# jianwang-mpi/GlobalEgoMocap

Hardware: AMD Instinct MI355X
Metric: optimised windows/sec (10-frame, 15-joint) (higher is better)
Workload: dtype f32

## Files before the change

globalegomocap_amd/csrc/gemm_f32.hip:

```cpp
#include <cstdio>
#include <cstdlib>

#include "gem_internal.h"
#include "gemm_glds.h"
#include "gemm_rows.h"

namespace gem {

typedef float f32x16 __attribute__((ext_vector_type(16)));
typedef float f32x4 __attribute__((ext_vector_type(4)));
typedef int i32x8 __attribute__((ext_vector_type(8)));

constexpr int BK_MIN = 32;

#ifdef GEM_TRACE
__device__ long long* g_gemm_trace = nullptr;
#define GEM_TRACE_MARK(slot_)                                                                            \
    if (g_gemm_trace && threadIdx.x == 0)                                                                \
        g_gemm_trace[4 * (blockIdx.x + gridDim.x * (blockIdx.y + gridDim.y * blockIdx.z)) + (slot_)] = wall_clock64();
#else
#define GEM_TRACE_MARK(slot_)
#endif

template <int TAPS, int EPI, int RM, int RN, int TAG, int BK>
__global__ __launch_bounds__(256) void gemm_f32_kernel(const float* __restrict__ A, int lda,
                                                       const float* __restrict__ W,
                                                       const float* __restrict__ bias,
                                                       const float* __restrict__ aux, float* __restrict__ C,
                                                       int ldc, int M, int N, int K, int T, int tiles_per_slice,
                                                       size_t slab_stride, const int* __restrict__ m_dev,
                                                       const int* __restrict__ row_map, int dyn_W) {
    constexpr int BM = 64 * RM, BN = 64 * RN;
    constexpr int LDS_LD = BK + 4;
    constexpr int TPR = BK / 4;
    constexpr int RPP = 256 / TPR;
    constexpr int A_LD4 = BM / RPP;
    constexpr int B_LD4 = BN / RPP;
    extern __shared__ __attribute__((aligned(16))) float lds[];
    constexpr int BUF = (BM + BN) * LDS_LD;

    const int tid = threadIdx.x;
    const int lane = tid & 63, wave = tid >> 6;
    const int wm = wave >> 1, wn = wave & 1;
    GEM_TRACE_MARK(0);
    int m0 = blockIdx.y * BM, n0 = blockIdx.x * BN;
    if (m_dev) M = *m_dev;
    const int kTiles = K / BK;
    bool split = gridDim.z > 1;
    int kt_begin = blockIdx.z * tiles_per_slice;
    int kt_end = min(TAPS * kTiles, kt_begin + tiles_per_slice);
    if (dyn_W > 0) {
        if (M <= 0) return;
        const int CT = N / BN;
        const DynSplit d = dyn_split(M, BM, CT, dyn_W, TAPS * kTiles, ldc);
        const int id = blockIdx.x + gridDim.x * (blockIdx.y + gridDim.y * blockIdx.z);
        if (id >= CT * d.RT * d.SK) return;
        const int ks = id / (CT * d.RT);
        n0 = (id % CT) * BN;
        m0 = ((id / CT) % d.RT) * BM;
        kt_begin = ks * d.per;
        kt_end = min(TAPS * kTiles, kt_begin + d.per);
        split = true;
        C += (size_t)ks * d.slab;
    } else {
        if (m0 >= M) return;
        if (split) C += (size_t)blockIdx.z * slab_stride;
    }

    const int c4 = (tid % TPR) * 4;
    const int lrow = tid / TPR;
    static_assert(A_LD4 <= 8, "row tables hold up to 8 entries");
    i32x8 a_row, a_t, a_src;
#pragma unroll
    for (int i = 0; i < A_LD4; ++i) {
        const int r_ = m0 + lrow + RPP * i;
        a_row[i] = r_;
        a_t[i] = (TAPS == 3) ? (r_ % T) : 0;
        int s_ = r_;
        if (TAPS == 1 && row_map) s_ = row_map[r_ < M ? r_ : 0];
        a_src[i] = s_;
    }
    f32x4 ra[A_LD4], rb[B_LD4];
    bool a_ok[A_LD4];

#define GEM_LOAD_TILE(kt_)                                                                                   \
    {                                                                                                        \
        const int tap_ = (TAPS == 3) ? ((kt_) >= kTiles) + ((kt_) >= 2 * kTiles) : 0;                                                      \
        const int k0_ = ((kt_) - tap_ * kTiles) * BK + c4;                                                   \
        _Pragma("unroll") for (int i = 0; i < A_LD4; ++i) {                                                  \
            bool ok_ = a_row[i] < M;                                                                         \
            if (TAPS == 3) {                                                                                 \
                const int tt_ = a_t[i] + tap_ - 1;                                                           \
                ok_ = ok_ && tt_ >= 0 && tt_ < T;                                                            \
            }                                                                                                \
            const int src_ = ok_ ? a_src[i] + ((TAPS == 3) ? tap_ - 1 : 0) : 0;                               \
            ra[i] = *reinterpret_cast<const f32x4*>(A + (size_t)src_ * lda + k0_);                           \
            a_ok[i] = ok_;   \
        }                                                                                                    \
        const float* Wt_ = W + (size_t)tap_ * N * K;                                                         \
        _Pragma("unroll") for (int i = 0; i < B_LD4; ++i)                                                    \
            rb[i] = *reinterpret_cast<const f32x4*>(Wt_ + (size_t)(n0 + lrow + RPP * i) * K + k0_);          \
    }
#define GEM_STORE_TILE(buf_)                                                                                 \
    {                                                                                                        \
        _Pragma("unroll") for (int i = 0; i < A_LD4; ++i)                                                    \
            *reinterpret_cast<f32x4*>(lds + (buf_) * BUF + (lrow + RPP * i) * LDS_LD + c4) =                  \
                a_ok[i] ? ra[i] : f32x4{0.f, 0.f, 0.f, 0.f};                                                 \
        _Pragma("unroll") for (int i = 0; i < B_LD4; ++i)                                                    \
            *reinterpret_cast<f32x4*>(lds + (buf_) * BUF + (BM + lrow + RPP * i) * LDS_LD + c4) = rb[i];      \
    }

    f32x16 acc[RM][RN];
#pragma unroll
    for (int i = 0; i < RM; ++i)
#pragma unroll
        for (int j = 0; j < RN; ++j)
#pragma unroll
            for (int e = 0; e < 16; ++e) acc[i][j][e] = 0.f;

    const int fr = lane & 31, fh = lane >> 5;
    constexpr bool DBUF = (RM * RN > 1);
    GEM_LOAD_TILE(kt_begin);
    GEM_STORE_TILE(0);
    __syncthreads();
    GEM_TRACE_MARK(1);
    int cur = 0;
#ifndef GEM_ABLATE
#define GEM_ABLATE 0
#endif
    for (int kt = kt_begin; kt < kt_end; ++kt) {
        const bool more = kt + 1 < kt_end;
        if (more && GEM_ABLATE < 1) GEM_LOAD_TILE(kt + 1);
        const float* as = lds + cur * BUF + (wm * 32 * RM + fr) * LDS_LD + fh * (BK / 2);
        const float* bs = lds + cur * BUF + (BM + wn * 32 * RN + fr) * LDS_LD + fh * (BK / 2);
        if (RM * RN == 1 && GEM_ABLATE == 0) {
            f32x4 av[BK / 8], bv[BK / 8];
#pragma unroll
            for (int q = 0; q < BK / 8; ++q) {
                av[q] = *reinterpret_cast<const f32x4*>(as + 4 * q);
                bv[q] = *reinterpret_cast<const f32x4*>(bs + 4 * q);
            }
            __builtin_amdgcn_sched_barrier(0);
#pragma unroll
            for (int q = 0; q < BK / 8; ++q) {
                acc[0][0] = __builtin_amdgcn_mfma_f32_32x32x2f32(av[q].x, bv[q].x, acc[0][0], 0, 0, 0);
                acc[0][0] = __builtin_amdgcn_mfma_f32_32x32x2f32(av[q].y, bv[q].y, acc[0][0], 0, 0, 0);
                acc[0][0] = __builtin_amdgcn_mfma_f32_32x32x2f32(av[q].z, bv[q].z, acc[0][0], 0, 0, 0);
                acc[0][0] = __builtin_amdgcn_mfma_f32_32x32x2f32(av[q].w, bv[q].w, acc[0][0], 0, 0, 0);
            }
        } else {
#pragma unroll
        for (int q = 0; q < BK / 8; ++q) {
            f32x4 av[RM], bv[RN];
#pragma unroll
            for (int i = 0; i < RM; ++i) av[i] = *reinterpret_cast<const f32x4*>(as + i * 32 * LDS_LD + 4 * (GEM_ABLATE >= 3 ? 0 : q));
#pragma unroll
            for (int j = 0; j < RN; ++j) bv[j] = *reinterpret_cast<const f32x4*>(bs + j * 32 * LDS_LD + 4 * (GEM_ABLATE >= 3 ? 0 : q));
            if (GEM_ABLATE >= 3) {
#pragma unroll
                for (int i = 0; i < RM; ++i) asm volatile("" : "+v"(av[i]));
            }
#pragma unroll
            for (int i = 0; i < RM; ++i)
#pragma unroll
                for (int j = 0; j < RN; ++j) {
                    acc[i][j] = __builtin_amdgcn_mfma_f32_32x32x2f32(av[i].x, bv[j].x, acc[i][j], 0, 0, 0);
                    acc[i][j] = __builtin_amdgcn_mfma_f32_32x32x2f32(av[i].y, bv[j].y, acc[i][j], 0, 0, 0);
                    acc[i][j] = __builtin_amdgcn_mfma_f32_32x32x2f32(av[i].z, bv[j].z, acc[i][j], 0, 0, 0);
                    acc[i][j] = __builtin_amdgcn_mfma_f32_32x32x2f32(av[i].w, bv[j].w, acc[i][j], 0, 0, 0);
                }
        }
        }
        if (GEM_ABLATE >= 2) continue;
        if (DBUF) {
            if (more) GEM_STORE_TILE(cur ^ 1);
            __syncthreads();
            cur ^= 1;
        } else {
            __syncthreads();
            if (more) GEM_STORE_TILE(0);
            __syncthreads();
        }
    }
#undef GEM_LOAD_TILE
#undef GEM_STORE_TILE
    GEM_TRACE_MARK(2);

#pragma unroll
    for (int i = 0; i < RM; ++i)
#pragma unroll
        for (int j = 0; j < RN; ++j) {
            const int col = n0 + wn * 32 * RN + j * 32 + fr;
            float bv = 0.f;
            if ((EPI == EPI_BIAS || EPI == EPI_BIAS_LRELU) && !split) bv = bias[col];
#pragma unroll
            for (int e = 0; e < 16; ++e) {
                const int row = m0 + wm * 32 * RM + i * 32 + (e & 3) + 8 * (e >> 2) + 4 * fh;
                if (row < M) {
                    float v = acc[i][j][e] + bv;
                    if (EPI == EPI_BIAS_LRELU && !split) v = v > 0.f ? v : v * LEAKY_SLOPE;
                    if (EPI == EPI_MASK && !split) v *= (aux[(size_t)row * ldc + col] > 0.f) ? 1.f : LEAKY_SLOPE;
                    C[(size_t)row * ldc + col] = v;
                }
            }
        }
    GEM_TRACE_MARK(3);
}

template <int EPI>
__global__ __launch_bounds__(256) void splitk_reduce_kernel(const float* __restrict__ slabs, int nslab, size_t slab_stride,
                                                            const float* __restrict__ bias, const float* __restrict__ aux,
                                                            float* __restrict__ C, int M, int N, int ldc,
                                                            const int* __restrict__ m_dev, int dyn_W, int n_tiles) {
    if (m_dev) M = *m_dev;
    if (dyn_W > 0) {
        const DynSplit d = dyn_split(M, 64, N / 64, dyn_W, n_tiles, ldc);
        nslab = d.SK;
        slab_stride = d.slab;
    }
    const int n4 = N / 4;
    const size_t i = (size_t)blockIdx.x * 256 + threadIdx.x;
    if (i >= (size_t)M * n4) return;
    const int row = (int)(i / n4), c = (int)(i - (size_t)row * n4) * 4;
    const size_t off = (size_t)row * ldc + c;
    f32x4 v = *reinterpret_cast<const f32x4*>(slabs + off);
    for (int z = 1; z < nslab; ++z) v += *reinterpret_cast<const f32x4*>(slabs + (size_t)z * slab_stride + off);
    if (EPI == EPI_BIAS || EPI == EPI_BIAS_LRELU) v += *reinterpret_cast<const f32x4*>(bias + c);
    if (EPI == EPI_BIAS_LRELU) {
#pragma unroll
        for (int q = 0; q < 4; ++q) v[q] = v[q] > 0.f ? v[q] : v[q] * LEAKY_SLOPE;
    }
    if (EPI == EPI_MASK) {
        const f32x4 m = *reinterpret_cast<const f32x4*>(aux + off);
#pragma unroll
        for (int q = 0; q < 4; ++q) v[q] *= m[q] > 0.f ? 1.f : LEAKY_SLOPE;
    }
    *reinterpret_cast<f32x4*>(C + off) = v;
}

constexpr int LDS_PER_CU = 160 * 1024;
int pick_splitk(const gem_handle* h, long blocks, int n_tiles, size_t slab_elems) {
    const int N_CU = h->n_cu;
    if (!h->ws.splitk || blocks >= 3 * N_CU) return 1;
    int best = 1;
    double best_score = -1.0;
    for (int sk = 1; sk <= 8; ++sk) {
        if (sk > 1 && (n_tiles / sk < 6 || (size_t)sk * slab_elems > h->ws.splitk_elems)) break;
        const long wgs = blocks * sk;
        const long per_cu = (wgs + N_CU - 1) / N_CU;
        double score = (double)wgs / (double)(per_cu * N_CU);
        if (per_cu < 2) score *= 0.6;
        score -= 0.01 * sk;
        if (score > best_score) { best_score = score; best = sk; }
    }
    return best;
}

int launch_splitk_reduce(gem_handle* h, int epi, int nslab, size_t slab, const float* bias, const float* aux, float* C, int M, int N,
                         int ldc, const int* m_dev, hipStream_t s, int dyn_W, int n_tiles) {
    const size_t n4 = (size_t)M * (N / 4);
    const dim3 grid((unsigned)((n4 + 255) / 256));
    switch (epi) {
        case EPI_BIAS: hipLaunchKernelGGL(splitk_reduce_kernel<EPI_BIAS>, grid, dim3(256), 0, s, h->ws.splitk, nslab, slab, bias, aux, C, M, N, ldc, m_dev, dyn_W, n_tiles); break;
        case EPI_BIAS_LRELU: hipLaunchKernelGGL(splitk_reduce_kernel<EPI_BIAS_LRELU>, grid, dim3(256), 0, s, h->ws.splitk, nslab, slab, bias, aux, C, M, N, ldc, m_dev, dyn_W, n_tiles); break;
        case EPI_MASK: hipLaunchKernelGGL(splitk_reduce_kernel<EPI_MASK>, grid, dim3(256), 0, s, h->ws.splitk, nslab, slab, bias, aux, C, M, N, ldc, m_dev, dyn_W, n_tiles); break;
        default: hipLaunchKernelGGL(splitk_reduce_kernel<EPI_NONE>, grid, dim3(256), 0, s, h->ws.splitk, nslab, slab, bias, aux, C, M, N, ldc, m_dev, dyn_W, n_tiles); break;
    }
    GEM_HIP(hipGetLastError());
    return 0;
}

template <int TAPS, int EPI, int RM, int RN, int TAG, int BK>
static int launch_one(gem_handle* h, const Layer& L, const float* A, int lda, const float* aux, float* C, int ldc, int M, int T,
                      hipStream_t s, const int* row_map) {
    const int* m_dev = h->ws.dyn ? h->ws.n_active + (TAPS == 3 ? 1 : 0) : nullptr;
    constexpr int BM = 64 * RM, BN = 64 * RN;
    size_t shmem = (RM * RN > 1 ? 2 : 1) * (size_t)(BM + BN) * (BK + 4) * sizeof(float);
    auto k = gemm_f32_kernel<TAPS, EPI, RM, RN, TAG, BK>;
    static PerDeviceOnce attr_once;
    if (attr_once.need(h->cfg.device)) {
        GEM_HIP(hipFuncSetAttribute(reinterpret_cast<const void*>(k), hipFuncAttributeMaxDynamicSharedMemorySize, LDS_PER_CU));
    }
    const int n_tiles = TAPS * (L.K / BK);
    dim3 grid(L.N / BN, (M + BM - 1) / BM, 1);
    const size_t slab = (size_t)M * ldc;
    const int sk = pick_splitk(h, (long)grid.x * grid.y, n_tiles, slab);
    const int per = (n_tiles + sk - 1) / sk;
    grid.z = (n_tiles + per - 1) / per;
    const long wgs = (long)grid.x * grid.y * grid.z;
    const long per_cu = (wgs + h->n_cu - 1) / h->n_cu;
    if (per_cu <= 8) {
        const size_t want = (((size_t)LDS_PER_CU - 8192) / per_cu) & ~(size_t)1023;
        if (want > shmem) shmem = want;
    }
    const bool dyn = m_dev && RM * RN == 1 && grid.z > 1 && (size_t)wgs * 64 * BN <= h->ws.splitk_elems;
    if (grid.z == 1) {
        note_kernel(h, reinterpret_cast<const void*>(k));
        hipLaunchKernelGGL(k, grid, dim3(256), shmem, s, A, lda, L.w, L.bias, aux, C, ldc, M, L.N, L.K, T, n_tiles, (size_t)0, m_dev,
                           row_map, 0);
        GEM_HIP(hipGetLastError());
        return 0;
    }
    note_kernel(h, reinterpret_cast<const void*>(k));
    hipLaunchKernelGGL(k, grid, dim3(256), shmem, s, A, lda, L.w, L.bias, aux, h->ws.splitk, ldc, M, L.N, L.K, T, per, slab, m_dev,
                       row_map, dyn ? (int)wgs : 0);
    GEM_HIP(hipGetLastError());
    if (h->ws.defer_reduce && BM == 64) {
        SlabSrc& d = h->ws.deferred;
        d.base = h->ws.splitk; d.nslab = (int)grid.z; d.stride = slab;
        d.dyn_W = dyn ? (int)wgs : 0; d.n_tiles = n_tiles; d.ldc = ldc; d.CT = L.N / BN; d.m_dev = m_dev;
        return 0;
    }
    return launch_splitk_reduce(h, EPI, (int)grid.z, slab, L.bias, aux, C, M, L.N, ldc, m_dev, s, dyn ? (int)wgs : 0, n_tiles);
}

template <int TAPS, int EPI>
static int launch_glds_f32(gem_handle* h, const Layer& L, const float* A, int lda, const float* aux, float* C, int ldc, int M, int T,
                           hipStream_t s, const int* row_map) {
    constexpr int BM = 128, BN = 128;
    auto k = glds::gemm_glds_kernel<true, TAPS, EPI, BM, BN, false, 16>;
    constexpr size_t smem = (size_t)BM * BN * 4;
    static PerDeviceOnce once;
    if (once.need(h->cfg.device))
        GEM_HIP(hipFuncSetAttribute(reinterpret_cast<const void*>(k), hipFuncAttributeMaxDynamicSharedMemorySize, LDS_PER_CU));
    glds::Args a{};
    a.A = A; a.W = L.w; a.bias = L.bias; a.aux = aux; a.C = C; a.zero16 = h->ws.zero16;
    a.m_dev = h->ws.dyn ? h->ws.n_active + (TAPS == 3 ? 1 : 0) : nullptr;
    a.row_map = row_map;
    a.lda = lda; a.ldc = ldc; a.M = M; a.N = L.N; a.K = L.K; a.T = T;
    a.n_split = 1; a.tiles_per_split = TAPS * (L.K / 32); a.slab_stride = 0;
    const int grid = ((M + BM - 1) / BM) * (L.N / BN);
    note_kernel(h, reinterpret_cast<const void*>(k));
    hipLaunchKernelGGL(k, dim3(grid), dim3(256), smem, s, a);
    GEM_HIP(hipGetLastError());
    return 0;
}

template <int S, int RT, bool FUSE>
static int launch_rows_as(gem_handle* h, const Layer& L, const float* A, int lda, float* C, int ldc, int M, hipStream_t s,
                          const int* row_map, const rows::Plan& p, bool direct, bool with_bias, bool lrelu) {
    auto k = rows::gemm_rows_kernel<S, RT, FUSE>;
    static PerDeviceOnce once;
    if (once.need(h->cfg.device))
        GEM_HIP(hipFuncSetAttribute(reinterpret_cast<const void*>(k), hipFuncAttributeMaxDynamicSharedMemorySize,
                                    S * rows::Geometry<RT>::STAGE_BYTES));
    Workspace& w = h->ws;
    rows::Args a{};
    a.A = A; a.W = L.w; a.bias = direct && with_bias ? L.bias : nullptr; a.lrelu = lrelu ? 1 : 0; a.C = direct ? C : w.splitk;
    a.m_dev = w.dyn ? w.n_active : nullptr;
    a.row_map = row_map;
    a.lda = lda; a.ldc = ldc; a.M = M; a.N = L.N; a.K = L.K;
    a.n_rb = p.n_rb; a.n_split = p.n_split; a.tiles_per_split = p.per; a.slab_stride = (size_t)M * ldc;
    if (FUSE) {
        a.phase_arr = w.phase; a.n_windows = M; a.done_phase = w.done_phase; a.T = h->T;
        a.perm_out = w.perm; a.slot_of_out = w.slot_of; a.n_active_out = w.n_active; a.log_slot = w.fuse_log;
    }
    const int grid = p.n_rb * (L.N / rows::BN) * p.n_split;
    note_kernel(h, reinterpret_cast<const void*>(k));
    hipLaunchKernelGGL(k, dim3(grid), dim3(256), (size_t)S * rows::Geometry<RT>::STAGE_BYTES, s, a);
    GEM_HIP(hipGetLastError());
    return 0;
}

static bool rows_plan(const gem_handle* h, const Layer& L, int lda, int ldc, int M, bool slabs, rows::Plan* out, bool* use8) {
    if (M < 48 || L.N % rows::BN != 0 || L.K % rows::BK != 0 || (size_t)h->ws.Bmax * lda * 4 >= ((size_t)1 << 32) ||
        (size_t)L.N * L.K * 4 >= ((size_t)1 << 32))
        return false;
    const rows::Plan p5 = rows::plan(M, L.N, L.K, 5, h->n_cu, slabs, h->ws.splitk_elems, ldc);
    const rows::Plan p8 = rows::plan(M, L.N, L.K, 8, h->n_cu, slabs, h->ws.splitk_elems, ldc);
    *use8 = p8.n_rb > 0 && (p5.n_rb == 0 || p8.cost < p5.cost - 1e-9);
    *out = *use8 ? p8 : p5;
    return out->n_rb != 0 && out->fill >= 0.75;
}

bool rows_can_fuse_compaction(const gem_handle* h, const Layer& L, int lda, int ldc, int B, bool slabs) {
    static const bool off = dev_env("GEM_NO_FUSED_COMPACT") != nullptr;
    rows::Plan p;
    bool use8;
    return !off && h->precision == GEM_PRECISION_F32 && B <= rows::FUSE_MAX_WINDOWS &&
           rows_plan(h, L, lda, ldc, B, slabs && h->ws.splitk, &p, &use8);
}

template <int EPI>
static int launch_rows(gem_handle* h, const Layer& L, const float* A, int lda, const float* aux, float* C, int ldc, int M,
                       hipStream_t s, const int* row_map) {
    const bool slabs = h->ws.defer_reduce && h->ws.splitk;
    rows::Plan p;
    bool use8;
    if (!rows_plan(h, L, lda, ldc, M, slabs, &p, &use8)) return -1;
    const bool direct = p.n_split == 1;
    if (!direct) {
        SlabSrc& d = h->ws.deferred;
        d.base = h->ws.splitk; d.nslab = p.n_split; d.stride = (size_t)M * ldc;
        d.dyn_W = 0; d.n_tiles = 0; d.ldc = ldc; d.CT = L.N / 64; d.m_dev = h->ws.dyn ? h->ws.n_active : nullptr;
    }
    (void)aux;
    constexpr bool with_bias = EPI != EPI_NONE, lrelu = EPI == EPI_BIAS_LRELU;
    if (h->ws.fuse_compact) {
        h->ws.fuse_compact = false;
        if (!row_map || M > rows::FUSE_MAX_WINDOWS) { set_error("launch_rows: fused compaction on a launch that cannot carry it"); return 1; }
        return use8 ? launch_rows_as<3, 8, true>(h, L, A, lda, C, ldc, M, s, row_map, p, direct, with_bias, lrelu)
                    : launch_rows_as<4, 5, true>(h, L, A, lda, C, ldc, M, s, row_map, p, direct, with_bias, lrelu);
    }
    return use8 ? launch_rows_as<3, 8, false>(h, L, A, lda, C, ldc, M, s, row_map, p, direct, with_bias, lrelu)
                : launch_rows_as<4, 5, false>(h, L, A, lda, C, ldc, M, s, row_map, p, direct, with_bias, lrelu);
}

template <int TAPS, int EPI, int TAG>
static int launch_tile(gem_handle* h, const Layer& L, const float* A, int lda, const float* aux, float* C, int ldc, int M, int T,
                       hipStream_t s, const int* row_map) {
    if (TAPS == 1 && (EPI == EPI_BIAS || EPI == EPI_NONE || EPI == EPI_BIAS_LRELU)) {
        const int rc = launch_rows<EPI>(h, L, A, lda, aux, C, ldc, M, s, row_map);
        if (rc >= 0) return rc;
    }
    if (L.N % 128 == 0 && L.K % 32 == 0 && (long)((M + 127) / 128) * (L.N / 128) >= 3L * h->n_cu / 2 && h->ws.zero16 &&
        !h->ws.defer_reduce)
        return launch_glds_f32<TAPS, EPI>(h, L, A, lda, aux, C, ldc, M, T, s, row_map);
    const long big_blocks = (long)((M + 127) / 128) * (L.N / 128);
    if (L.N % 128 == 0 && big_blocks >= 512) return launch_one<TAPS, EPI, 2, 2, TAG, 32>(h, L, A, lda, aux, C, ldc, M, T, s, row_map);
    return launch_one<TAPS, EPI, 1, 1, TAG, 32>(h, L, A, lda, aux, C, ldc, M, T, s, row_map);
}

int launch_gemm(gem_handle* h, const Layer& L, int epi, const float* A, int lda, const float* aux, float* C, int ldc, int M,
                int T, hipStream_t s, int family, const int* row_map) {
    if (L.K % BK_MIN != 0 || L.N % 64 != 0 || lda % 4 != 0) {
        set_error("launch_gemm: dimensions must be padded (K%32, N%64, lda%4)");
        return 1;
    }
    if (M <= 0) return 0;
    h->ws.deferred = SlabSrc{};
    Profile::Rec rec;
    const bool prof = h->prof.on && family >= 0;
    if (prof) {
        GEM_HIP(hipEventCreate(&rec.a));
        GEM_HIP(hipEventCreate(&rec.b));
        rec.family = family;
        rec.flops = 2.0 * M * (double)L.N * L.K * L.taps;
        if (h->ws.dyn && L.taps == 1) {
            rec.log_idx = h->ws.cur_log;
            rec.flops_per_window = 2.0 * (double)L.N * L.K;
        }
        GEM_HIP(hipEventRecord(rec.a, s));
    }
    int rc = 1;
    if (h->precision != GEM_PRECISION_F32 && L.wb_hi && (h->precision == GEM_PRECISION_BF16 || L.wb_lo)) {
        rc = launch_gemm_bf16(h, L, epi, h->precision == GEM_PRECISION_BF16 ? 1 : 3, A, lda, aux, C, ldc, M, T, s, row_map);
    } else if (L.taps == 1) {
        if (family == 0 && epi == EPI_BIAS) rc = launch_tile<1, EPI_BIAS, 1>(h, L, A, lda, aux, C, ldc, M, T, s, row_map);
        else if (epi == EPI_BIAS) rc = launch_tile<1, EPI_BIAS, 0>(h, L, A, lda, aux, C, ldc, M, T, s, row_map);
        else if (epi == EPI_NONE) rc = launch_tile<1, EPI_NONE, 0>(h, L, A, lda, aux, C, ldc, M, T, s, row_map);
        else if (epi == EPI_BIAS_LRELU) rc = launch_tile<1, EPI_BIAS_LRELU, 1>(h, L, A, lda, aux, C, ldc, M, T, s, row_map);
        else set_error("launch_gemm: unsupported epilogue for a linear layer");
    } else if (L.taps == 3) {
        if (epi == EPI_BIAS) rc = launch_tile<3, EPI_BIAS, 0>(h, L, A, lda, aux, C, ldc, M, T, s, row_map);
        else if (epi == EPI_BIAS_LRELU) rc = launch_tile<3, EPI_BIAS_LRELU, 0>(h, L, A, lda, aux, C, ldc, M, T, s, row_map);
        else if (epi == EPI_MASK) rc = launch_tile<3, EPI_MASK, 0>(h, L, A, lda, aux, C, ldc, M, T, s, row_map);
        else if (epi == EPI_NONE) rc = launch_tile<3, EPI_NONE, 0>(h, L, A, lda, aux, C, ldc, M, T, s, row_map);
    } else {
        set_error("launch_gemm: taps must be 1 or 3");
    }
    if (rc) return rc;
    if (prof) {
        GEM_HIP(hipEventRecord(rec.b, s));
        h->prof.recs.push_back(rec);
    }
    commit_kernel_names(h, prof ? family : -1);
    return 0;
}

}
```

globalegomocap_amd/csrc/gemm_rows.h:

```cpp
#pragma once
#include <hip/hip_runtime.h>
#include <stdint.h>
#include <type_traits>

namespace gem {
namespace rows {

typedef float f32x4 __attribute__((ext_vector_type(4)));

constexpr int BN = 64;
constexpr int BK = 64;
constexpr int ROW_BYTES = BK * 4;

struct Args {
    const float* A;
    const float* W;
    const float* bias;
    int lrelu;
    float* C;
    const int* m_dev;
    const int* row_map;
    int lda, ldc, M, N, K;
    const int* phase_arr;
    int n_windows, done_phase, T;
    int* perm_out;
    int* slot_of_out;
    int* n_active_out;
    int* log_slot;
    int n_rb;
    int n_split, tiles_per_split;
    size_t slab_stride;
};

template <int RT>
struct Geometry {
    static constexpr int A_BYTES = RT * 16 * ROW_BYTES, B_BYTES = BN * ROW_BYTES, STAGE_BYTES = A_BYTES + B_BYTES;
    static constexpr int A_INSTR = A_BYTES / 1024 / 4, B_INSTR = B_BYTES / 1024 / 4;
    static constexpr int PIECES = A_INSTR + B_INSTR;
    static_assert(A_BYTES % 4096 == 0, "the A tile must split into whole DMA pieces per wave");
};

#ifndef GEM_ROWS_ABLATE
#define GEM_ROWS_ABLATE 0
#endif

#ifdef GEM_ROWS_CLOCK
__device__ long long g_rows_clock[6];
#endif

constexpr int FUSE_MAX_WINDOWS = 512;

template <int S, int RT, bool FUSE = false>
__device__ __forceinline__ void gemm_rows_body(const Args& a) {
    typedef Geometry<RT> G;
    static_assert(S >= 3 && S * G::STAGE_BYTES <= 160 * 1024, "ring must fit the LDS");
    static_assert(4 * RT * 4096 <= S * G::STAGE_BYTES, "the four partial tiles are reduced through the ring's LDS");
    extern __shared__ __attribute__((aligned(16))) unsigned char smem[];
    const int tid = threadIdx.x, lane = tid & 63;
    const int wave = __builtin_amdgcn_readfirstlane(tid >> 6);
#ifdef GEM_ROWS_CLOCK
    const long long w_begin = wall_clock64();
#endif

    const int n_ct = a.N / BN;
    const int total = n_ct * a.n_split * a.n_rb;
    const int id = blockIdx.x;
    if (id >= total) return;
    const int q8 = total >> 3, r8 = total & 7, x8 = id & 7, k8 = id >> 3;
    const int pid = (x8 < r8 ? x8 * (q8 + 1) : r8 * (q8 + 1) + (x8 - r8) * q8) + k8;
    const int rb = pid % a.n_rb;
    const int ks = (pid / a.n_rb) % a.n_split;
    const int ct = pid / (a.n_rb * a.n_split);
    const int n0 = ct * BN;
    const int kTiles = a.K / BK;
    const int kt_begin = ks * a.tiles_per_split, kt_end = min(kTiles, kt_begin + a.tiles_per_split);
    const int nk = kt_end - kt_begin;
    if (nk <= 0) return;

    const int lrow = lane >> 4, lchunk = lane & 15;
    unsigned b_off[G::B_INSTR];
#pragma unroll
    for (int j = 0; j < G::B_INSTR; ++j) {
        const int r = (wave * G::B_INSTR + j) * 4 + lrow;
        b_off[j] = (unsigned)r * (unsigned)a.K * 4u + (unsigned)((lchunk ^ (r & 15)) * 16);
    }
    const unsigned char* b_base = reinterpret_cast<const unsigned char*>(a.W + (size_t)n0 * a.K) + (size_t)kt_begin * ROW_BYTES;
#pragma unroll
    for (int i = 0; i < S - 1; ++i) {
        unsigned char* lb = smem + i * G::STAGE_BYTES + G::A_BYTES + wave * (G::B_INSTR * 1024);
        const unsigned char* src = b_base + (size_t)min(i, nk - 1) * ROW_BYTES;
#pragma unroll
        for (int j = 0; j < G::B_INSTR; ++j)
            __builtin_amdgcn_global_load_lds((const __attribute__((address_space(1))) void*)(src + b_off[j]),
                                             (__attribute__((address_space(3))) void*)(lb + j * 1024), 16, 0, 0);
    }

    int M;
    __shared__ int s_perm[FUSE ? FUSE_MAX_WINDOWS : 1];
    __shared__ int s_wsum[4];
    if (FUSE) {
        int base = 0;
        for (int start = 0; start < a.n_windows; start += 256) {
            const int b = start + tid;
            const bool active = b < a.n_windows && a.phase_arr[b] != a.done_phase;
            const unsigned long long m = __ballot(active);
            const int prefix = __popcll(m & ((1ull << lane) - 1ull));
            if (lane == 0) s_wsum[wave] = __popcll(m);
            __syncthreads();
            int woff = 0, total = 0;
#pragma unroll
            for (int i = 0; i < 4; ++i) { if (i < wave) woff += s_wsum[i]; total += s_wsum[i]; }
            const int before = base + woff + prefix;
            if (active) s_perm[before] = b;
            if (blockIdx.x == 0 && b < a.n_windows) {
                if (active) { a.perm_out[before] = b; a.slot_of_out[b] = before; }
            }
            __syncthreads();
            base += total;
        }
        M = base;
        if (blockIdx.x == 0) {
            int fin = 0;
            for (int start = 0; start < a.n_windows; start += 256) {
                const int b = start + tid;
                const bool done = b < a.n_windows && a.phase_arr[b] == a.done_phase;
                const unsigned long long m = __ballot(done);
                const int prefix = __popcll(m & ((1ull << lane) - 1ull));
                __syncthreads();
                if (lane == 0) s_wsum[wave] = __popcll(m);
                __syncthreads();
                int woff = 0, total = 0;
#pragma unroll
                for (int i = 0; i < 4; ++i) { if (i < wave) woff += s_wsum[i]; total += s_wsum[i]; }
                if (done) { const int sl = M + fin + woff + prefix; a.perm_out[sl] = b; a.slot_of_out[b] = sl; }
                fin += total;
            }
            if (tid == 0) { a.n_active_out[0] = M; a.n_active_out[1] = M * a.T; *a.log_slot = M; }
        }
    } else {
        M = a.m_dev ? *a.m_dev : a.M;
    }
    const int R = (max(M, 0) + 15) >> 4;
    const int rpb = (R + a.n_rb - 1) / a.n_rb;
    const int t0 = rb * rpb;
    const int nrt = min(min(rpb, R - t0), RT);
    if (nrt <= 0) {
        asm volatile("s_waitcnt vmcnt(0)" ::: "memory");
        return;
    }
    const int m0 = t0 * 16;
    unsigned a_off[G::A_INSTR];
#pragma unroll
    for (int j = 0; j < G::A_INSTR; ++j) {
        const int r = (wave * G::A_INSTR + j) * 4 + lrow;
        int src = min(m0 + r, M - 1);
        if (FUSE) src = s_perm[src];
        else if (a.row_map) src = a.row_map[src];
        a_off[j] = (unsigned)src * (unsigned)a.lda * 4u + (unsigned)((lchunk ^ (r & 15)) * 16);
    }
    const unsigned char* a_base = reinterpret_cast<const unsigned char*>(a.A) + (size_t)kt_begin * ROW_BYTES;
#pragma unroll
    for (int i = 0; i < S - 1; ++i) {
        unsigned char* la = smem + i * G::STAGE_BYTES + wave * (G::A_INSTR * 1024);
        const unsigned char* src = a_base + (size_t)min(i, nk - 1) * ROW_BYTES;
#pragma unroll
        for (int j = 0; j < G::A_INSTR; ++j)
            __builtin_amdgcn_global_load_lds((const __attribute__((address_space(1))) void*)(src + a_off[j]),
                                             (__attribute__((address_space(3))) void*)(la + j * 1024), 16, 0, 0);
    }
    int staged = S - 1;
    a_base += (size_t)min(S - 1, nk - 1) * ROW_BYTES;
    b_base += (size_t)min(S - 1, nk - 1) * ROW_BYTES;
    auto stage = [&](int buf) {
        unsigned char* la = smem + buf * G::STAGE_BYTES + wave * (G::A_INSTR * 1024);
        unsigned char* lb = smem + buf * G::STAGE_BYTES + G::A_BYTES + wave * (G::B_INSTR * 1024);
#pragma unroll
        for (int j = 0; j < G::A_INSTR; ++j)
            __builtin_amdgcn_global_load_lds((const __attribute__((address_space(1))) void*)(a_base + a_off[j]),
                                             (__attribute__((address_space(3))) void*)(la + j * 1024), 16, 0, 0);
#pragma unroll
        for (int j = 0; j < G::B_INSTR; ++j)
            __builtin_amdgcn_global_load_lds((const __attribute__((address_space(1))) void*)(b_base + b_off[j]),
                                             (__attribute__((address_space(3))) void*)(lb + j * 1024), 16, 0, 0);
        ++staged;
        const int adv = staged < nk ? ROW_BYTES : 0;
        a_base += adv;
        b_base += adv;
    };

    const int fr = lane & 15, fh = lane >> 4;
    const int f_off = fr * ROW_BYTES + (((4 * wave + fh) ^ fr) << 4);
    const int col = n0 + 4 * fh;
    float* Cb = a.C + (a.n_split > 1 ? (size_t)ks * a.slab_stride : 0);

    auto body = [&](auto nrt_c) {
        constexpr int NRT = decltype(nrt_c)::value;
        struct Frags { f32x4 w[4]; f32x4 a[NRT]; };
        f32x4 acc[4][NRT];
#pragma unroll
        for (int i = 0; i < 4; ++i)
#pragma unroll
            for (int j = 0; j < NRT; ++j) acc[i][j] = f32x4{0.f, 0.f, 0.f, 0.f};
        auto fetch = [&](Frags& f, int buf) {
            const unsigned char* base = smem + buf * G::STAGE_BYTES + f_off;
#pragma unroll
            for (int i = 0; i < 4; ++i) f.w[i] = *reinterpret_cast<const f32x4*>(base + G::A_BYTES + i * 16 * ROW_BYTES);
#pragma unroll
            for (int j = 0; j < NRT; ++j) f.a[j] = *reinterpret_cast<const f32x4*>(base + j * 16 * ROW_BYTES);
        };
        auto mfmas = [&](const Frags& f) {
#pragma unroll
            for (int e = 0; e < 4; ++e)
#pragma unroll
                for (int i = 0; i < 4; ++i)
#pragma unroll
                    for (int j = 0; j < NRT; ++j) acc[i][j] = __builtin_amdgcn_mfma_f32_16x16x4f32(f.w[i][e], f.a[j][e], acc[i][j], 0, 0, 0);
        };
        int cur = 0;
        auto step = [&](const Frags& f, Frags& g, auto wait_c) {
            const int nb = cur + 1 == S ? 0 : cur + 1;
            if (GEM_ROWS_ABLATE != 6) asm volatile("s_waitcnt vmcnt(%0)" ::"n"(decltype(wait_c)::value) : "memory");
            if (GEM_ROWS_ABLATE != 6) __builtin_amdgcn_s_barrier();
            if (GEM_ROWS_ABLATE != 3 && GEM_ROWS_ABLATE != 6) stage(cur == 0 ? S - 1 : cur - 1);
            if (GEM_ROWS_ABLATE != 1 && GEM_ROWS_ABLATE != 6) fetch(g, nb);
            if (GEM_ROWS_ABLATE != 2) mfmas(f);
#pragma unroll
            for (int i = 0; i < 16 * NRT; ++i) {
                __builtin_amdgcn_sched_group_barrier(0x008, 1, 0);
                __builtin_amdgcn_sched_group_barrier(0x126, 1, 0);
            }
            cur = nb;
        };
        static_assert(S == 3 || S == 4, "the peeled first step below is written for rings of 3 or 4");
        asm volatile("s_waitcnt vmcnt(%0)" ::"n"((S - 2) * G::A_INSTR) : "memory");
        __builtin_amdgcn_s_barrier();
        const std::integral_constant<int, (S - 3) * G::PIECES> steady;
        Frags f0, f1;
        fetch(f0, 0);
#ifdef GEM_ROWS_CLOCK
        if (GEM_ROWS_ABLATE == 6) f1 = f0;
        const long long c0 = clock64(), w0 = wall_clock64();
#endif
        if constexpr (S == 4) {
            step(f0, f1, std::integral_constant<int, G::A_INSTR>{});
            for (int t = 1; t < nk; t += 2) {
                step(f1, f0, steady);
                if (t + 1 < nk) step(f0, f1, steady);
            }
        } else {
            for (int t = 0; t < nk; t += 2) {
                step(f0, f1, steady);
                if (t + 1 < nk) step(f1, f0, steady);
            }
        }
#ifdef GEM_ROWS_CLOCK
        const long long w1 = wall_clock64();
        if (blockIdx.x == 8 && tid == 0) { g_rows_clock[0] = clock64() - c0; g_rows_clock[1] = w1 - w0; g_rows_clock[2] = w0 - w_begin; }
#endif
        asm volatile("s_waitcnt vmcnt(0)" ::: "memory");
        __syncthreads();
#pragma unroll
        for (int i = 0; i < 4; ++i)
#pragma unroll
            for (int j = 0; j < NRT; ++j)
                *reinterpret_cast<f32x4*>(smem + ((wave * 4 + i) * NRT + j) * 1024 + lane * 16) = acc[i][j];
        __syncthreads();
        f32x4 bv = {0.f, 0.f, 0.f, 0.f};
        if (a.n_split == 1 && a.bias) bv = *reinterpret_cast<const f32x4*>(a.bias + col + 16 * wave);
#pragma unroll
        for (int j = 0; j < NRT; ++j) {
            f32x4 v = *reinterpret_cast<const f32x4*>(smem + ((0 * 4 + wave) * NRT + j) * 1024 + lane * 16);
#pragma unroll
            for (int w = 1; w < 4; ++w) v += *reinterpret_cast<const f32x4*>(smem + ((w * 4 + wave) * NRT + j) * 1024 + lane * 16);
            const int row = m0 + j * 16 + fr;
            if (row < M) {
                v += bv;
                if (a.lrelu && a.n_split == 1) {
#pragma unroll
                    for (int e = 0; e < 4; ++e) v[e] = v[e] > 0.f ? v[e] : v[e] * 0.01f;
                }
                *reinterpret_cast<f32x4*>(Cb + (size_t)row * a.ldc + col + 16 * wave) = v;
            }
        }
#ifdef GEM_ROWS_CLOCK
        if (blockIdx.x == 8 && tid == 0) g_rows_clock[3] = wall_clock64() - w1;
#endif
    };
    switch (nrt) {
        case 1: body(std::integral_constant<int, 1>{}); break;
        case 2: body(std::integral_constant<int, (RT >= 2 ? 2 : RT)>{}); break;
        case 3: body(std::integral_constant<int, (RT >= 3 ? 3 : RT)>{}); break;
        case 4: body(std::integral_constant<int, (RT >= 4 ? 4 : RT)>{}); break;
        case 5: body(std::integral_constant<int, (RT >= 5 ? 5 : RT)>{}); break;
        case 6: body(std::integral_constant<int, (RT >= 6 ? 6 : RT)>{}); break;
        case 7: body(std::integral_constant<int, (RT >= 7 ? 7 : RT)>{}); break;
        default: body(std::integral_constant<int, RT>{}); break;
    }
}

template <int S, int RT, bool FUSE = false>
__global__ __launch_bounds__(256) void gemm_rows_kernel(const Args a) { gemm_rows_body<S, RT, FUSE>(a); }

struct Plan { int n_rb, n_split, per; double fill, cost; };
inline Plan plan(int M, int N, int K, int rt_max, int n_cu, bool allow_split, size_t slab_capacity_elems, int ldc) {
    Plan best{0, 0, 0, 0.0, 1e30};
    if (N % BN != 0 || K % BK != 0 || M <= 0) return best;
    const int R = (M + 15) / 16, n_ct = N / BN, nk = K / BK;
    double best_cost = 1e30;
    for (int n_rb = (R + rt_max - 1) / rt_max; n_rb <= R; ++n_rb) {
        const int rpb = (R + n_rb - 1) / n_rb;
        if (rpb < 3 && n_rb > (R + rt_max - 1) / rt_max) break;
        for (int sk = 1; sk <= (allow_split ? 8 : 1); ++sk) {
            if ((long)n_rb * n_ct * sk > n_cu) break;
            if (sk > 1 && (nk / sk < 4 || (size_t)sk * M * ldc > slab_capacity_elems)) break;
            const int per = (nk + sk - 1) / sk;
            const double slab_units = sk > 1 ? sk * ((double)M * N * 8.0 / 3.0e12) / 0.214e-6 : 0.0;
            const double cost = ((double)rpb + 0.7) * per + slab_units;
            if (cost < best_cost) { best_cost = cost; best = Plan{n_rb, sk, per, (double)R * n_ct * nk / ((double)n_cu * rpb * per), cost}; }
        }
    }
    return best;
}

}
}
```

Before: 31970.

## Add 32-column weight tiles to row GEMM and choose tile shape by cost model

The row-streaming GEMM kernel now takes the weight tile width (32 or 64 columns) as a template parameter. The A-tile DMA count is tied to the actual row count rather than the maximum, and the epilogue reduction is redistributed across waves. A new planner keeps the existing split-K choice, then searches over tile width and row-tile count to reduce wave quantisation and idle CUs on small-M layers. MFMA/DMA interleaving hints are also re-scheduled. The cost is more kernel instantiations and a heuristic cost model that may pick narrower tiles with less weight reuse.

```diff
diff --git a/globalegomocap_amd/csrc/gemm_f32.hip b/globalegomocap_amd/csrc/gemm_f32.hip
--- a/globalegomocap_amd/csrc/gemm_f32.hip
+++ b/globalegomocap_amd/csrc/gemm_f32.hip
@@ -336,14 +336,14 @@
     return 0;
 }
 
-template <int S, int RT, bool FUSE>
+template <int S, int RT, int BN, bool FUSE>
 static int launch_rows_as(gem_handle* h, const Layer& L, const float* A, int lda, float* C, int ldc, int M, hipStream_t s,
                           const int* row_map, const rows::Plan& p, bool direct, bool with_bias, bool lrelu) {
-    auto k = rows::gemm_rows_kernel<S, RT, FUSE>;
+    auto k = rows::gemm_rows_kernel<S, RT, BN, FUSE>;
     static PerDeviceOnce once;
     if (once.need(h->cfg.device))
         GEM_HIP(hipFuncSetAttribute(reinterpret_cast<const void*>(k), hipFuncAttributeMaxDynamicSharedMemorySize,
-                                    S * rows::Geometry<RT>::STAGE_BYTES));
+                                    S * rows::Geometry<RT, BN>::STAGE_BYTES));
     Workspace& w = h->ws;
     rows::Args a{};
     a.A = A; a.W = L.w; a.bias = direct && with_bias ? L.bias : nullptr; a.lrelu = lrelu ? 1 : 0; a.C = direct ? C : w.splitk;
@@ -355,30 +355,37 @@
         a.phase_arr = w.phase; a.n_windows = M; a.done_phase = w.done_phase; a.T = h->T;
         a.perm_out = w.perm; a.slot_of_out = w.slot_of; a.n_active_out = w.n_active; a.log_slot = w.fuse_log;
     }
-    const int grid = p.n_rb * (L.N / rows::BN) * p.n_split;
+    const int grid = p.n_rb * (L.N / BN) * p.n_split;
+    const size_t smem = (size_t)S * rows::Geometry<RT, BN>::STAGE_BYTES;
     note_kernel(h, reinterpret_cast<const void*>(k));
-    hipLaunchKernelGGL(k, dim3(grid), dim3(256), (size_t)S * rows::Geometry<RT>::STAGE_BYTES, s, a);
+    hipLaunchKernelGGL(k, dim3(grid), dim3(256), smem, s, a);
     GEM_HIP(hipGetLastError());
     return 0;
 }
 
-static bool rows_plan(const gem_handle* h, const Layer& L, int lda, int ldc, int M, bool slabs, rows::Plan* out, bool* use8) {
-    if (M < 48 || L.N % rows::BN != 0 || L.K % rows::BK != 0 || (size_t)h->ws.Bmax * lda * 4 >= ((size_t)1 << 32) ||
+template <bool FUSE>
+static int launch_rows_plan(gem_handle* h, const Layer& L, const float* A, int lda, float* C, int ldc, int M, hipStream_t s,
+                            const int* row_map, const rows::Plan& p, bool direct, bool with_bias, bool lrelu) {
+    if (p.bn == 32)
+        return p.rt == 8 ? launch_rows_as<3, 8, 32, FUSE>(h, L, A, lda, C, ldc, M, s, row_map, p, direct, with_bias, lrelu)
+                         : launch_rows_as<4, 5, 32, FUSE>(h, L, A, lda, C, ldc, M, s, row_map, p, direct, with_bias, lrelu);
+    return p.rt == 8 ? launch_rows_as<3, 8, 64, FUSE>(h, L, A, lda, C, ldc, M, s, row_map, p, direct, with_bias, lrelu)
+                     : launch_rows_as<4, 5, 64, FUSE>(h, L, A, lda, C, ldc, M, s, row_map, p, direct, with_bias, lrelu);
+}
+
+static bool rows_plan(const gem_handle* h, const Layer& L, int lda, int ldc, int M, bool slabs, rows::Plan* out) {
+    if (M < 48 || L.N % 64 != 0 || L.K % rows::BK != 0 || (size_t)h->ws.Bmax * lda * 4 >= ((size_t)1 << 32) ||
         (size_t)L.N * L.K * 4 >= ((size_t)1 << 32))
         return false;
-    const rows::Plan p5 = rows::plan(M, L.N, L.K, 5, h->n_cu, slabs, h->ws.splitk_elems, ldc);
-    const rows::Plan p8 = rows::plan(M, L.N, L.K, 8, h->n_cu, slabs, h->ws.splitk_elems, ldc);
-    *use8 = p8.n_rb > 0 && (p5.n_rb == 0 || p8.cost < p5.cost - 1e-9);
-    *out = *use8 ? p8 : p5;
-    return out->n_rb != 0 && out->fill >= 0.75;
+    *out = rows::choose(M, L.N, L.K, h->n_cu, slabs, h->ws.splitk_elems, ldc);
+    return out->n_rb != 0;
 }
 
 bool rows_can_fuse_compaction(const gem_handle* h, const Layer& L, int lda, int ldc, int B, bool slabs) {
     static const bool off = dev_env("GEM_NO_FUSED_COMPACT") != nullptr;
     rows::Plan p;
-    bool use8;
     return !off && h->precision == GEM_PRECISION_F32 && B <= rows::FUSE_MAX_WINDOWS &&
-           rows_plan(h, L, lda, ldc, B, slabs && h->ws.splitk, &p, &use8);
+           rows_plan(h, L, lda, ldc, B, slabs && h->ws.splitk, &p);
 }
 
 template <int EPI>
@@ -386,8 +393,7 @@
                        hipStream_t s, const int* row_map) {
     const bool slabs = h->ws.defer_reduce && h->ws.splitk;
     rows::Plan p;
-    bool use8;
-    if (!rows_plan(h, L, lda, ldc, M, slabs, &p, &use8)) return -1;
+    if (!rows_plan(h, L, lda, ldc, M, slabs, &p)) return -1;
     const bool direct = p.n_split == 1;
     if (!direct) {
         SlabSrc& d = h->ws.deferred;
@@ -399,11 +405,9 @@
     if (h->ws.fuse_compact) {
         h->ws.fuse_compact = false;
         if (!row_map || M > rows::FUSE_MAX_WINDOWS) { set_error("launch_rows: fused compaction on a launch that cannot carry it"); return 1; }
-        return use8 ? launch_rows_as<3, 8, true>(h, L, A, lda, C, ldc, M, s, row_map, p, direct, with_bias, lrelu)
-                    : launch_rows_as<4, 5, true>(h, L, A, lda, C, ldc, M, s, row_map, p, direct, with_bias, lrelu);
-    }
-    return use8 ? launch_rows_as<3, 8, false>(h, L, A, lda, C, ldc, M, s, row_map, p, direct, with_bias, lrelu)
-                : launch_rows_as<4, 5, false>(h, L, A, lda, C, ldc, M, s, row_map, p, direct, with_bias, lrelu);
+        return launch_rows_plan<true>(h, L, A, lda, C, ldc, M, s, row_map, p, direct, with_bias, lrelu);
+    }
+    return launch_rows_plan<false>(h, L, A, lda, C, ldc, M, s, row_map, p, direct, with_bias, lrelu);
 }
 
 template <int TAPS, int EPI, int TAG>
diff --git a/globalegomocap_amd/csrc/gemm_rows.h b/globalegomocap_amd/csrc/gemm_rows.h
--- a/globalegomocap_amd/csrc/gemm_rows.h
+++ b/globalegomocap_amd/csrc/gemm_rows.h
@@ -8,7 +8,6 @@
 
 typedef float f32x4 __attribute__((ext_vector_type(4)));
 
-constexpr int BN = 64;
 constexpr int BK = 64;
 constexpr int ROW_BYTES = BK * 4;
 
@@ -32,12 +31,12 @@
     size_t slab_stride;
 };
 
-template <int RT>
+template <int RT, int BN>
 struct Geometry {
+    static_assert(BN == 32 || BN == 64, "weight tiles of 32 or 64 columns");
+    static constexpr int NI = BN / 16;
     static constexpr int A_BYTES = RT * 16 * ROW_BYTES, B_BYTES = BN * ROW_BYTES, STAGE_BYTES = A_BYTES + B_BYTES;
-    static constexpr int A_INSTR = A_BYTES / 1024 / 4, B_INSTR = B_BYTES / 1024 / 4;
-    static constexpr int PIECES = A_INSTR + B_INSTR;
-    static_assert(A_BYTES % 4096 == 0, "the A tile must split into whole DMA pieces per wave");
+    static constexpr int B_INSTR = B_BYTES / 1024 / 4;
 };
 
 #ifndef GEM_ROWS_ABLATE
@@ -50,11 +49,13 @@
 
 constexpr int FUSE_MAX_WINDOWS = 512;
 
-template <int S, int RT, bool FUSE = false>
+template <int S, int RT, int BN, bool FUSE = false>
 __device__ __forceinline__ void gemm_rows_body(const Args& a) {
-    typedef Geometry<RT> G;
+    typedef Geometry<RT, BN> G;
+    constexpr int NI = G::NI;
     static_assert(S >= 3 && S * G::STAGE_BYTES <= 160 * 1024, "ring must fit the LDS");
-    static_assert(4 * RT * 4096 <= S * G::STAGE_BYTES, "the four partial tiles are reduced through the ring's LDS");
+    static_assert(4 * NI * RT * 1024 <= S * G::STAGE_BYTES, "the four partial tiles are reduced through the ring's LDS");
+    static_assert(4 * NI >= 2 * (1 + G::B_INSTR), "two MFMAs in front of every DMA piece of a step");
     extern __shared__ __attribute__((aligned(16))) unsigned char smem[];
     const int tid = threadIdx.x, lane = tid & 63;
     const int wave = __builtin_amdgcn_readfirstlane(tid >> 6);
@@ -94,6 +95,7 @@
             __builtin_amdgcn_global_load_lds((const __attribute__((address_space(1))) void*)(src + b_off[j]),
                                              (__attribute__((address_space(3))) void*)(lb + j * 1024), 16, 0, 0);
     }
+    b_base += (size_t)min(S - 1, nk - 1) * ROW_BYTES;
 
     int M;
     __shared__ int s_perm[FUSE ? FUSE_MAX_WINDOWS : 1];
@@ -149,44 +151,6 @@
         return;
     }
     const int m0 = t0 * 16;
-    unsigned a_off[G::A_INSTR];
-#pragma unroll
-    for (int j = 0; j < G::A_INSTR; ++j) {
-        const int r = (wave * G::A_INSTR + j) * 4 + lrow;
-        int src = min(m0 + r, M - 1);
-        if (FUSE) src = s_perm[src];
-        else if (a.row_map) src = a.row_map[src];
-        a_off[j] = (unsigned)src * (unsigned)a.lda * 4u + (unsigned)((lchunk ^ (r & 15)) * 16);
-    }
-    const unsigned char* a_base = reinterpret_cast<const unsigned char*>(a.A) + (size_t)kt_begin * ROW_BYTES;
-#pragma unroll
-    for (int i = 0; i < S - 1; ++i) {
-        unsigned char* la = smem + i * G::STAGE_BYTES + wave * (G::A_INSTR * 1024);
-        const unsigned char* src = a_base + (size_t)min(i, nk - 1) * ROW_BYTES;
-#pragma unroll
-        for (int j = 0; j < G::A_INSTR; ++j)
-            __builtin_amdgcn_global_load_lds((const __attribute__((address_space(1))) void*)(src + a_off[j]),
-                                             (__attribute__((address_space(3))) void*)(la + j * 1024), 16, 0, 0);
-    }
-    int staged = S - 1;
-    a_base += (size_t)min(S - 1, nk - 1) * ROW_BYTES;
-    b_base += (size_t)min(S - 1, nk - 1) * ROW_BYTES;
-    auto stage = [&](int buf) {
-        unsigned char* la = smem + buf * G::STAGE_BYTES + wave * (G::A_INSTR * 1024);
-        unsigned char* lb = smem + buf * G::STAGE_BYTES + G::A_BYTES + wave * (G::B_INSTR * 1024);
-#pragma unroll
-        for (int j = 0; j < G::A_INSTR; ++j)
-            __builtin_amdgcn_global_load_lds((const __attribute__((address_space(1))) void*)(a_base + a_off[j]),
-                                             (__attribute__((address_space(3))) void*)(la + j * 1024), 16, 0, 0);
-#pragma unroll
-        for (int j = 0; j < G::B_INSTR; ++j)
-            __builtin_amdgcn_global_load_lds((const __attribute__((address_space(1))) void*)(b_base + b_off[j]),
-                                             (__attribute__((address_space(3))) void*)(lb + j * 1024), 16, 0, 0);
-        ++staged;
-        const int adv = staged < nk ? ROW_BYTES : 0;
-        a_base += adv;
-        b_base += adv;
-    };
 
     const int fr = lane & 15, fh = lane >> 4;
     const int f_off = fr * ROW_BYTES + (((4 * wave + fh) ^ fr) << 4);
@@ -195,16 +159,57 @@
 
     auto body = [&](auto nrt_c) {
         constexpr int NRT = decltype(nrt_c)::value;
-        struct Frags { f32x4 w[4]; f32x4 a[NRT]; };
-        f32x4 acc[4][NRT];
-#pragma unroll
-        for (int i = 0; i < 4; ++i)
+        constexpr int A_INSTR = NRT;
+        constexpr int PIECES = A_INSTR + G::B_INSTR;
+        unsigned a_off[A_INSTR];
+#pragma unroll
+        for (int j = 0; j < A_INSTR; ++j) {
+            const int r = (wave * A_INSTR + j) * 4 + lrow;
+            int src = min(m0 + r, M - 1);
+            if (FUSE) src = s_perm[src];
+            else if (a.row_map) src = a.row_map[src];
+            a_off[j] = (unsigned)src * (unsigned)a.lda * 4u + (unsigned)((lchunk ^ (r & 15)) * 16);
+        }
+        const unsigned char* a_base = reinterpret_cast<const unsigned char*>(a.A) + (size_t)kt_begin * ROW_BYTES;
+#pragma unroll
+        for (int i = 0; i < S - 1; ++i) {
+            unsigned char* la = smem + i * G::STAGE_BYTES + wave * (A_INSTR * 1024);
+            const unsigned char* src = a_base + (size_t)min(i, nk - 1) * ROW_BYTES;
+#pragma unroll
+            for (int j = 0; j < A_INSTR; ++j)
+                __builtin_amdgcn_global_load_lds((const __attribute__((address_space(1))) void*)(src + a_off[j]),
+                                                 (__attribute__((address_space(3))) void*)(la + j * 1024), 16, 0, 0);
+        }
+        int staged = S - 1;
+        a_base += (size_t)min(S - 1, nk - 1) * ROW_BYTES;
+        const unsigned char* bb = b_base;
+        auto stage = [&](int buf) {
+            unsigned char* la = smem + buf * G::STAGE_BYTES + wave * (A_INSTR * 1024);
+            unsigned char* lb = smem + buf * G::STAGE_BYTES + G::A_BYTES + wave * (G::B_INSTR * 1024);
+#pragma unroll
+            for (int j = 0; j < A_INSTR; ++j)
+                __builtin_amdgcn_global_load_lds((const __attribute__((address_space(1))) void*)(a_base + a_off[j]),
+                                                 (__attribute__((address_space(3))) void*)(la + j * 1024), 16, 0, 0);
+#pragma unroll
+            for (int j = 0; j < G::B_INSTR; ++j)
+                __builtin_amdgcn_global_load_lds((const __attribute__((address_space(1))) void*)(bb + b_off[j]),
+                                                 (__attribute__((address_space(3))) void*)(lb + j * 1024), 16, 0, 0);
+            ++staged;
+            const int adv = staged < nk ? ROW_BYTES : 0;
+            a_base += adv;
+            bb += adv;
+        };
+
+        struct Frags { f32x4 w[NI]; f32x4 a[NRT]; };
+        f32x4 acc[NI][NRT];
+#pragma unroll
+        for (int i = 0; i < NI; ++i)
 #pragma unroll
             for (int j = 0; j < NRT; ++j) acc[i][j] = f32x4{0.f, 0.f, 0.f, 0.f};
         auto fetch = [&](Frags& f, int buf) {
             const unsigned char* base = smem + buf * G::STAGE_BYTES + f_off;
 #pragma unroll
-            for (int i = 0; i < 4; ++i) f.w[i] = *reinterpret_cast<const f32x4*>(base + G::A_BYTES + i * 16 * ROW_BYTES);
+            for (int i = 0; i < NI; ++i) f.w[i] = *reinterpret_cast<const f32x4*>(base + G::A_BYTES + i * 16 * ROW_BYTES);
 #pragma unroll
             for (int j = 0; j < NRT; ++j) f.a[j] = *reinterpret_cast<const f32x4*>(base + j * 16 * ROW_BYTES);
         };
@@ -212,7 +217,7 @@
 #pragma unroll
             for (int e = 0; e < 4; ++e)
 #pragma unroll
-                for (int i = 0; i < 4; ++i)
+                for (int i = 0; i < NI; ++i)
 #pragma unroll
                     for (int j = 0; j < NRT; ++j) acc[i][j] = __builtin_amdgcn_mfma_f32_16x16x4f32(f.w[i][e], f.a[j][e], acc[i][j], 0, 0, 0);
         };
@@ -225,16 +230,22 @@
             if (GEM_ROWS_ABLATE != 1 && GEM_ROWS_ABLATE != 6) fetch(g, nb);
             if (GEM_ROWS_ABLATE != 2) mfmas(f);
 #pragma unroll
-            for (int i = 0; i < 16 * NRT; ++i) {
+            for (int i = 0; i < PIECES; ++i) {
+                __builtin_amdgcn_sched_group_barrier(0x008, 2, 0);
+                __builtin_amdgcn_sched_group_barrier(0x006, 2, 0);
+                __builtin_amdgcn_sched_group_barrier(0x020, 1, 0);
+            }
+#pragma unroll
+            for (int i = 0; i < 4 * NI * NRT - 2 * PIECES; ++i) {
                 __builtin_amdgcn_sched_group_barrier(0x008, 1, 0);
-                __builtin_amdgcn_sched_group_barrier(0x126, 1, 0);
+                __builtin_amdgcn_sched_group_barrier(0x106, 1, 0);
             }
             cur = nb;
         };
         static_assert(S == 3 || S == 4, "the peeled first step below is written for rings of 3 or 4");
-        asm volatile("s_waitcnt vmcnt(%0)" ::"n"((S - 2) * G::A_INSTR) : "memory");
+        asm volatile("s_waitcnt vmcnt(%0)" ::"n"((S - 2) * A_INSTR) : "memory");
         __builtin_amdgcn_s_barrier();
-        const std::integral_constant<int, (S - 3) * G::PIECES> steady;
+        const std::integral_constant<int, (S - 3) * PIECES> steady;
         Frags f0, f1;
         fetch(f0, 0);
 #ifdef GEM_ROWS_CLOCK
@@ -242,7 +253,7 @@
         const long long c0 = clock64(), w0 = wall_clock64();
 #endif
         if constexpr (S == 4) {
-            step(f0, f1, std::integral_constant<int, G::A_INSTR>{});
+            step(f0, f1, std::integral_constant<int, A_INSTR>{});
             for (int t = 1; t < nk; t += 2) {
                 step(f1, f0, steady);
                 if (t + 1 < nk) step(f0, f1, steady);
@@ -260,18 +271,21 @@
         asm volatile("s_waitcnt vmcnt(0)" ::: "memory");
         __syncthreads();
 #pragma unroll
-        for (int i = 0; i < 4; ++i)
+        for (int i = 0; i < NI; ++i)
 #pragma unroll
             for (int j = 0; j < NRT; ++j)
-                *reinterpret_cast<f32x4*>(smem + ((wave * 4 + i) * NRT + j) * 1024 + lane * 16) = acc[i][j];
+                *reinterpret_cast<f32x4*>(smem + ((wave * NI + i) * NRT + j) * 1024 + lane * 16) = acc[i][j];
         __syncthreads();
-        f32x4 bv = {0.f, 0.f, 0.f, 0.f};
-        if (a.n_split == 1 && a.bias) bv = *reinterpret_cast<const f32x4*>(a.bias + col + 16 * wave);
-#pragma unroll
-        for (int j = 0; j < NRT; ++j) {
-            f32x4 v = *reinterpret_cast<const f32x4*>(smem + ((0 * 4 + wave) * NRT + j) * 1024 + lane * 16);
-#pragma unroll
-            for (int w = 1; w < 4; ++w) v += *reinterpret_cast<const f32x4*>(smem + ((w * 4 + wave) * NRT + j) * 1024 + lane * 16);
+#pragma unroll
+        for (int q = 0; q < (NI * NRT + 3) / 4; ++q) {
+            const int blk = 4 * q + wave;
+            if (NI * NRT % 4 != 0 && blk >= NI * NRT) break;
+            const int i = blk / NRT, j = blk % NRT;
+            f32x4 bv = {0.f, 0.f, 0.f, 0.f};
+            if (a.n_split == 1 && a.bias) bv = *reinterpret_cast<const f32x4*>(a.bias + col + 16 * i);
+            f32x4 v = *reinterpret_cast<const f32x4*>(smem + ((0 * NI + i) * NRT + j) * 1024 + lane * 16);
+#pragma unroll
+            for (int w = 1; w < 4; ++w) v += *reinterpret_cast<const f32x4*>(smem + ((w * NI + i) * NRT + j) * 1024 + lane * 16);
             const int row = m0 + j * 16 + fr;
             if (row < M) {
                 v += bv;
@@ -279,7 +293,7 @@
 #pragma unroll
                     for (int e = 0; e < 4; ++e) v[e] = v[e] > 0.f ? v[e] : v[e] * 0.01f;
                 }
-                *reinterpret_cast<f32x4*>(Cb + (size_t)row * a.ldc + col + 16 * wave) = v;
+                *reinterpret_cast<f32x4*>(Cb + (size_t)row * a.ldc + col + 16 * i) = v;
             }
         }
 #ifdef GEM_ROWS_CLOCK
@@ -298,12 +312,13 @@
     }
 }
 
-template <int S, int RT, bool FUSE = false>
-__global__ __launch_bounds__(256) void gemm_rows_kernel(const Args a) { gemm_rows_body<S, RT, FUSE>(a); }
-
-struct Plan { int n_rb, n_split, per; double fill, cost; };
-inline Plan plan(int M, int N, int K, int rt_max, int n_cu, bool allow_split, size_t slab_capacity_elems, int ldc) {
-    Plan best{0, 0, 0, 0.0, 1e30};
+template <int S, int RT, int BN, bool FUSE = false>
+__global__ __launch_bounds__(256) void gemm_rows_kernel(const Args a) { gemm_rows_body<S, RT, BN, FUSE>(a); }
+
+struct Plan { int n_rb, n_split, per, bn, rt; double fill, cost; };
+inline Plan slices(int M, int N, int K, int rt_max, int n_cu, bool allow_split, size_t slab_capacity_elems, int ldc) {
+    constexpr int BN = 64;
+    Plan best{0, 0, 0, BN, rt_max, 0.0, 1e30};
     if (N % BN != 0 || K % BK != 0 || M <= 0) return best;
     const int R = (M + 15) / 16, n_ct = N / BN, nk = K / BK;
     double best_cost = 1e30;
@@ -316,11 +331,45 @@
             const int per = (nk + sk - 1) / sk;
             const double slab_units = sk > 1 ? sk * ((double)M * N * 8.0 / 3.0e12) / 0.214e-6 : 0.0;
             const double cost = ((double)rpb + 0.7) * per + slab_units;
-            if (cost < best_cost) { best_cost = cost; best = Plan{n_rb, sk, per, (double)R * n_ct * nk / ((double)n_cu * rpb * per), cost}; }
+            if (cost < best_cost) { best_cost = cost; best = Plan{n_rb, sk, per, BN, rt_max, (double)R * n_ct * nk / ((double)n_cu * rpb * per), cost}; }
         }
     }
     return best;
 }
 
-}
-}
+constexpr double STEP_OVERHEAD = 0.7;
+
+inline Plan tile(int M, int N, int K, int n_split, int per, int bn, int rt_max, int n_cu) {
+    Plan best{0, n_split, per, bn, rt_max, 0.0, 1e30};
+    if (N % bn != 0 || M <= 0) return best;
+    const int R = (M + 15) / 16, n_ct = N / bn, nk = K / BK;
+    for (int n_rb = (R + rt_max - 1) / rt_max; n_rb <= R; ++n_rb) {
+        const int rpb = (R + n_rb - 1) / n_rb;
+        if ((n_rb - 1) * rpb >= R) continue;
+        const long wgs = (long)n_rb * n_ct * n_split;
+        const int waves = (int)((wgs + n_cu - 1) / n_cu);
+        const double cost = waves * ((double)rpb * bn / 64.0 + STEP_OVERHEAD) * per;
+        const double fill = (double)R * (N / 64.0) * nk / ((double)n_cu * waves * rpb * (bn / 64.0) * per);
+        if (cost < best.cost - 1e-9) best = Plan{n_rb, n_split, per, bn, rt_max, fill, cost};
+        if (waves > 1) break;
+    }
+    return best;
+}
+
+inline Plan choose(int M, int N, int K, int n_cu, bool allow_split, size_t slab_capacity_elems, int ldc) {
+    const Plan p5 = slices(M, N, K, 5, n_cu, allow_split, slab_capacity_elems, ldc);
+    const Plan p8 = slices(M, N, K, 8, n_cu, allow_split, slab_capacity_elems, ldc);
+    const bool use8 = p8.n_rb > 0 && (p5.n_rb == 0 || p8.cost < p5.cost - 1e-9);
+    const Plan s = use8 ? p8 : p5;
+    Plan best{0, 0, 0, 0, 0, 0.0, 1e30};
+    if (s.n_rb == 0 || s.fill < 0.75) return best;
+    const int cand[4][2] = {{64, 5}, {64, 8}, {32, 5}, {32, 8}};
+    for (const auto& c : cand) {
+        const Plan t = tile(M, N, K, s.n_split, s.per, c[0], c[1], n_cu);
+        if (t.n_rb > 0 && t.cost < best.cost - 1e-9) best = t;
+    }
+    return best;
+}
+
+}
+}
```

Measured after the change: 32330, median of 6. +1.1%, better.
